# edogariu/artist-style-transfer

Measured on NVIDIA B200. Metric: train_images_per_sec_256, higher is better.
Workload: dtype bf16

## Files before the change

### artist_style_transfer_b200/csrc/common.cuh

```cuda
#pragma once
#include <cstring>
#include <cstdlib>
#include <cuda_runtime.h>
#include <cuda_bf16.h>
#include <cuda_fp16.h>
#include <stdint.h>
#include <stdio.h>
#include <atomic>

#include "../../include/ast.h"

namespace ast {

void set_error(const char* fmt, ...);
extern std::atomic<long long> g_launches;
inline void count_launch(int n = 1) { g_launches.fetch_add(n, std::memory_order_relaxed); }

enum Family {
  FAM_CONV_TC = 0, FAM_CONV_PX, FAM_CONV_WS, FAM_CONV_HX, FAM_CONV_SIMT, FAM_WGRAD_TC, FAM_WGRAD_THIN, FAM_WGRAD_SIMT, FAM_GRAM_TC,
  FAM_GRAM_SIMT, FAM_IN_APPLY, FAM_IN_BWD, FAM_IN_STATS, FAM_POOL, FAM_MSE, FAM_POINTWISE, FAM_OPTIM, FAM_CONV_ST, FAM_COUNT
};
void count_work(int family, double flops, double bytes);
inline double esize(const ast_image* im) { return im->dtype == AST_F32 ? 4.0 : (im->dtype == AST_U8 ? 1.0 : 2.0); }
inline double img_bytes(const ast_image* im) { return im ? (double)im->n * im->h * im->w * im->c * esize(im) : 0.0; }
// ... 62 lines not shown
  static constexpr int id = AST_BF16;
  __device__ static __forceinline__ float ld(const __nv_bfloat16* p) { return __bfloat162float(*p); }
  __device__ static __forceinline__ void st(__nv_bfloat16* p, float v) { *p = __float2bfloat16_rn(v); }
};

__device__ __forceinline__ __half f2h_sat(float v) { return __float2half_rn(fminf(fmaxf(v, -65504.f), 65504.f)); }
template <bool F16>
__device__ __forceinline__ unsigned pack2(float a, float b) {
  if (F16) { const __half2 h = __halves2half2(f2h_sat(a), f2h_sat(b)); return *reinterpret_cast<const unsigned*>(&h); }
  const __nv_bfloat162 h = __floats2bfloat162_rn(a, b);
  return *reinterpret_cast<const unsigned*>(&h);
}
__device__ __forceinline__ unsigned pack2_16(int dtype, float a, float b) { return dtype == AST_F16 ? pack2<true>(a, b) : pack2<false>(a, b); }
__device__ __forceinline__ float ld_elem(const Img& im, long long off) {
  if (im.dtype == AST_F32) return ((const float*)im.ptr)[off];
  if (im.dtype == AST_U8) return (float)((const unsigned char*)im.ptr)[off];
  if (im.dtype == AST_BF16) return __bfloat162float(((const __nv_bfloat16*)im.ptr)[off]);
  return __half2float(((const __half*)im.ptr)[off]);
}
__device__ __forceinline__ void st_elem(const Img& im, long long off, float v) {
  if (im.dtype == AST_F32) ((float*)im.ptr)[off] = v;
  else if (im.dtype == AST_BF16) ((__nv_bfloat16*)im.ptr)[off] = __float2bfloat16_rn(v);
  else if (im.dtype == AST_F16) ((__half*)im.ptr)[off] = f2h_sat(v);
  else ((unsigned char*)im.ptr)[off] = (unsigned char)__float2uint_rz(fminf(fmaxf(v, 0.f), 255.f));
}
__device__ __forceinline__ long long img_off(const Img& im, int n, int y, int x, int c) {
  return (long long)n * im.sn + (long long)y * im.sh + (long long)x * im.sw + (long long)c * im.sc;
}
__device__ __forceinline__ int reflect_idx(int i, int n) {
  if (i < 0) i = -i;
  if (i >= n) i = 2 * (n - 1) - i;
  return i;
}
template <typename F>
__device__ __forceinline__ void reflect_fold_border(int pad, int H, int W, int i, int j, F&& add) {
  const int r1 = (i >= 1 && i <= pad) ? pad - i : -1;
  const int r2 = (i <= H - 2 && i >= H - 1 - pad) ? pad + 2 * (H - 1) - i : -1;
  const int c1 = (j >= 1 && j <= pad) ? pad - j : -1;
  const int c2 = (j <= W - 2 && j >= W - 1 - pad) ? pad + 2 * (W - 1) - j : -1;
#pragma unroll
  for (int a_ = 0; a_ < 3; ++a_) {
    const int r = a_ == 0 ? i + pad : (a_ == 1 ? r1 : r2);
    if (r < 0) continue;
#pragma unroll
    for (int b_ = 0; b_ < 3; ++b_) {
      const int cc = b_ == 0 ? j + pad : (b_ == 1 ? c1 : c2);
      if (cc < 0 || (a_ == 0 && b_ == 0)) continue;
      add(r, cc);
    }
  }
}

__device__ __forceinline__ float warp_sum(float v) {
#pragma unroll
  for (int o = 16; o > 0; o >>= 1) v += __shfl_xor_sync(0xffffffffu, v, o);
  return v;
}

template <typename T> struct Vec16;
template <> struct Vec16<float> {
  static constexpr int N = 4;
  __device__ static __forceinline__ void load(const float* p, float* out) {
    float4 v = *reinterpret_cast<const float4*>(p);
    out[0] = v.x; out[1] = v.y; out[2] = v.z; out[3] = v.w;
  }
  __device__ static __forceinline__ void store(float* p, const float* in) {
    *reinterpret_cast<float4*>(p) = make_float4(in[0], in[1], in[2], in[3]);
  }
};
template <> struct Vec16<__nv_bfloat16> {
  static constexpr int N = 8;
  __device__ static __forceinline__ void load(const __nv_bfloat16* p, float* out) {
// ... 64 lines not shown
```

### artist_style_transfer_b200/csrc/norm.cu

```cuda
#include "tc_common.cuh"

namespace ast {

constexpr int NT = 256;

template <typename T>
__global__ void __launch_bounds__(NT)
in_stats_partial_kernel(Img x, float* __restrict__ ws, int nblk, int chunk) {
  constexpr int VEC = Vec16<T>::N;
  extern __shared__ float sm[];
  const int C = x.c, lanes = C / VEC, slots = NT / lanes;
  const int tid = threadIdx.x, lane = tid % lanes, slot = tid / lanes;
  const int n = blockIdx.y, blk = blockIdx.x;
  const int hw = x.h * x.w;
  const int pbeg = blk * chunk, pend = min(hw, pbeg + chunk);
  const T* base = (const T*)x.ptr + (long long)n * x.sn + lane * VEC;

  float k[VEC], s1[VEC], s2[VEC];
#pragma unroll
  for (int e = 0; e < VEC; ++e) { k[e] = 0.f; s1[e] = 0.f; s2[e] = 0.f; }
  int cnt = 0;
  if (slot < slots) {
    for (int p = pbeg + slot; p < pend; p += slots) {
      const int y = p / x.w, xx = p - y * x.w;
// ... 55 lines not shown
    rstd[n * C + c] = rsqrtf(qa / (float)hw + eps);
  }
}

__global__ void in_finalize_kernel(const double* __restrict__ sums, int total, double inv_hw, float eps,
                                   float* __restrict__ mean, float* __restrict__ rstd) {
  const int i = blockIdx.x * blockDim.x + threadIdx.x;
  if (i >= total) return;
  const double m = sums[2 * i] * inv_hw;
  const double var = fmax(sums[2 * i + 1] * inv_hw - m * m, 0.0);
  mean[i] = (float)m;
  rstd[i] = (float)(1.0 / sqrt(var + (double)eps));
}


constexpr int NS_CONSUMER_WARPS = 8;
constexpr int NS_CONSUMERS = NS_CONSUMER_WARPS * 32;
constexpr int NS_THREADS = NS_CONSUMERS + 32;
constexpr int NS_SLAB_MAX = 16384;
constexpr int NS_MAX_STAGES = 8;
constexpr int NS_SMEM_BUDGET = 100 * 1024;

struct Rows {
  char* ptr;
  long long sn;
  int sh;
};

struct NsShape {
  int C, H, W, pad;
  int nblk;
  int seg, nseg;
  int stages, slab_bytes;
};

template <typename T> struct NsVec;
template <> struct NsVec<float> {
  static constexpr int N = 4;
  __device__ static __forceinline__ void unpack(const uint4& r, float* v) {
    v[0] = __uint_as_float(r.x); v[1] = __uint_as_float(r.y); v[2] = __uint_as_float(r.z); v[3] = __uint_as_float(r.w);
  }
  __device__ static __forceinline__ uint4 pack(const float* v) {
    return make_uint4(__float_as_uint(v[0]), __float_as_uint(v[1]), __float_as_uint(v[2]), __float_as_uint(v[3]));
  }
};
template <> struct NsVec<__nv_bfloat16> {
  static constexpr int N = 8;
  __device__ static __forceinline__ void unpack(const uint4& r, float* v) {
    const unsigned w[4] = {r.x, r.y, r.z, r.w};
#pragma unroll
    for (int i = 0; i < 4; ++i) { v[2 * i] = __uint_as_float(w[i] << 16); v[2 * i + 1] = __uint_as_float(w[i] & 0xffff0000u); }
  }
  __device__ static __forceinline__ uint4 pack(const float* v) {
    uint4 r;
    __nv_bfloat162* h = reinterpret_cast<__nv_bfloat162*>(&r);
#pragma unroll
    for (int i = 0; i < 4; ++i) h[i] = __floats2bfloat162_rn(v[2 * i], v[2 * i + 1]);
    return r;
  }
};

template <int VEC>
__device__ __forceinline__ void ns_ldc(const float* __restrict__ p, float* v) {
#pragma unroll
  for (int e = 0; e < VEC; e += 4) {
    const float4 t = __ldg(reinterpret_cast<const float4*>(p + e));
// ... 86 lines not shown
  for (int k = 0; k < nunits; ++k) {
    const int s = k % sh.stages;
    const unsigned ph = (unsigned)(k / sh.stages) & 1u;
    const int oy = rbeg + k / sh.nseg, sg = k % sh.nseg;
    const int oa = sg * sh.seg, ob = min(OW, oa + sh.seg);
    int xa, xb;
    apply_span(oa, ob, sh.pad, sh.W, xa, xb);
    const unsigned xs = buf + s * stage_bytes + (unsigned)(c * (int)sizeof(T));
    const int orow = oy * (out.sh / VEC);
    mbar_wait(&full[s], ph);
    for (int ox = oa + slot; ox < ob; ox += slots) {
      const int j = reflect_idx(ox - sh.pad, sh.W) - xa;
      float v[VEC];
      NsVec<T>::unpack(lds128(xs + (unsigned)(j * C * (int)sizeof(T))), v);
#pragma unroll
      for (int e = 0; e < VEC; ++e) v[e] = fmaf(A[e], v[e], D[e]);
      if (res.ptr) {
        float r[VEC];
        NsVec<T>::unpack(lds128(xs + sh.slab_bytes + (unsigned)(j * C * (int)sizeof(T))), r);
#pragma unroll
        for (int e = 0; e < VEC; ++e) v[e] += r[e];
      }
      if (relu) {
#pragma unroll
        for (int e = 0; e < VEC; ++e) v[e] = fmaxf(v[e], 0.f);
      }
      oimg[orow + ox * lanes] = NsVec<T>::pack(v);
    }
    __syncwarp();
    if ((threadIdx.x & 31) == 0) mbar_arrive(&empty[s]);
  }
}

template <typename T, int VEC>
__device__ __forceinline__ void ns_fold_border(const T* gimg, int gsh, int C, int pad, int H, int W, int i, int j, float* g) {
  reflect_fold_border(pad, H, W, i, j, [&](int r, int cc) {
    float t[VEC];
    NsVec<T>::unpack(__ldg(reinterpret_cast<const uint4*>(gimg + (r * gsh + cc * C))), t);
#pragma unroll
    for (int e = 0; e < VEC; ++e) g[e] += t[e];
  });
}

template <typename T>
__device__ __forceinline__ void ns_bwd_produce(const Rows& x, const Rows& gpad, const Rows& gextra, const NsShape& sh, int n,
                                               int rbeg, int nunits, int k0, unsigned buf, int stage_bytes,
                                               unsigned long long* full, unsigned long long* empty) {
  const int C = sh.C;
  const int nslabs = 1 + (gpad.ptr ? 1 : 0) + (gextra.ptr ? 1 : 0);
  for (int k = 0; k < nunits; ++k) {
    const int s = (k0 + k) % sh.stages;
    const unsigned ph = (unsigned)((k0 + k) / sh.stages) & 1u;
    const int i = rbeg + k / sh.nseg, sg = k % sh.nseg;
    const int ja = sg * sh.seg, jb = min(sh.W, ja + sh.seg);
    const unsigned bytes = (unsigned)((jb - ja) * C * (int)sizeof(T));
    mbar_wait(&empty[s], ph ^ 1u);
    mbar_expect_tx(&full[s], bytes * nslabs);
    unsigned dst = buf + s * stage_bytes;
    bulk_load(dst, img_at<T>(x, n) + (i * x.sh + ja * C), bytes, &full[s]);
    dst += sh.slab_bytes;
    if (gpad.ptr) {
      bulk_load(dst, img_at<T>(gpad, n) + ((i + sh.pad) * gpad.sh + (ja + sh.pad) * C), bytes, &full[s]);
      dst += sh.slab_bytes;
    }
    if (gextra.ptr) bulk_load(dst, img_at<T>(gextra, n) + (i * gextra.sh + ja * C), bytes, &full[s]);
  }
}

template <typename T, int VEC>
__device__ __forceinline__ void ns_gprime(unsigned xs, unsigned gs, unsigned es, const T* gimg, int gsh, bool has_gextra,
                                          const NsShape& sh, bool brow, int i, int j, const float* A, const float* D,
                                          int relu, float* xv, float* g) {
  NsVec<T>::unpack(lds128(xs), xv);
  if (gimg) {
    NsVec<T>::unpack(lds128(gs), g);
    if (sh.pad > 0 && (brow || j <= sh.pad || j >= sh.W - 1 - sh.pad))
      ns_fold_border<T, VEC>(gimg, gsh, sh.C, sh.pad, sh.H, sh.W, i, j, g);
  } else {
#pragma unroll
    for (int e = 0; e < VEC; ++e) g[e] = 0.f;
  }
  if (has_gextra) {
    float t[VEC];
    NsVec<T>::unpack(lds128(es), t);
#pragma unroll
    for (int e = 0; e < VEC; ++e) g[e] += t[e];
  }
#pragma unroll
  for (int e = 0; e < VEC; ++e)
    if (relu && !(fmaf(A[e], xv[e], D[e]) > 0.f)) g[e] = 0.f;
}

enum NsMode { NS_STATS = 1, NS_APPLY = 2, NS_BOTH = 3 };

template <typename T, int MODE>
__global__ void __launch_bounds__(NS_THREADS, 2)
in_bwd_staged_kernel(Rows x, const float* __restrict__ mean, const float* __restrict__ rstd,
                     const float* __restrict__ gamma, const float* __restrict__ beta, Rows gpad, Rows gextra,
                     NsShape sh, int relu, float* __restrict__ s1, float* __restrict__ s2, int* __restrict__ arrive,
                     Rows dx, Rows gtotal) {
  constexpr int VEC = NsVec<T>::N;
  extern __shared__ unsigned char smem_raw[];
  __shared__ __align__(8) unsigned long long full[NS_MAX_STAGES], empty[NS_MAX_STAGES];
  const unsigned buf = (smem_u32(smem_raw) + 127u) & ~127u;
  ns_init(full, empty, sh.stages);
  const int n = blockIdx.y, C = sh.C;
  const int rbeg = (int)((long long)blockIdx.x * sh.H / sh.nblk), rend = (int)((long long)(blockIdx.x + 1) * sh.H / sh.nblk);
  const int nunits = (rend - rbeg) * sh.nseg;
  const int nslabs = 1 + (gpad.ptr ? 1 : 0) + (gextra.ptr ? 1 : 0);
  const int stage_bytes = nslabs * sh.slab_bytes;

  if (threadIdx.x >= NS_CONSUMERS) {
    if (threadIdx.x == NS_CONSUMERS) {
      ns_bwd_produce<T>(x, gpad, gextra, sh, n, rbeg, nunits, 0, buf, stage_bytes, full, empty);
      if (MODE == NS_BOTH) ns_bwd_produce<T>(x, gpad, gextra, sh, n, rbeg, nunits, nunits, buf, stage_bytes, full, empty);
    }
    return;
  }
  const int lanes = C / VEC, slots = NS_CONSUMERS / lanes;
  const int lane = threadIdx.x % lanes, slot = threadIdx.x / lanes;
  const int c = lane * VEC;
  float A[VEC], D[VEC];
  ns_fold_ad<VEC>(gamma, beta, mean, rstd, n, C, c, A, D);
  const T* const gimg = gpad.ptr ? img_at<T>(gpad, n) + c : nullptr;

  auto consume = [&](int k, int pos, auto&& f) {
    const int s = pos % sh.stages;
    const unsigned ph = (unsigned)(pos / sh.stages) & 1u;
    const int i = rbeg + k / sh.nseg, sg = k % sh.nseg;
    const int ja = sg * sh.seg, jb = min(sh.W, ja + sh.seg);
    const bool brow = sh.pad > 0 && (i <= sh.pad || i >= sh.H - 1 - sh.pad);
    const unsigned xs = buf + s * stage_bytes + (unsigned)(c * (int)sizeof(T));
    const unsigned gs = xs + sh.slab_bytes;
    const unsigned es = xs + (gpad.ptr ? 2 : 1) * sh.slab_bytes;
    mbar_wait(&full[s], ph);
    for (int j = ja + slot; j < jb; j += slots) {
      const unsigned poff = (unsigned)((j - ja) * C * (int)sizeof(T));
      float xv[VEC], g[VEC];
      ns_gprime<T, VEC>(xs + poff, gs + poff, es + poff, gimg, gpad.sh, gextra.ptr != nullptr, sh, brow, i, j, A, D, relu,
                        xv, g);
      f(j, xv, g);
    }
    __syncwarp();
    if ((threadIdx.x & 31) == 0) mbar_arrive(&empty[s]);
  };

  if (MODE & NS_STATS) {
    float t1[VEC], t2[VEC];
#pragma unroll
    for (int e = 0; e < VEC; ++e) { t1[e] = 0.f; t2[e] = 0.f; }
    for (int k = 0; k < nunits; ++k)
      consume(k, k, [&](int, const float* xv, const float* g) {
#pragma unroll
        for (int e = 0; e < VEC; ++e) { t1[e] += g[e]; t2[e] = fmaf(g[e], xv[e], t2[e]); }
      });
    float* r1 = reinterpret_cast<float*>(smem_raw + (buf - smem_u32(smem_raw)) +
                                         (MODE == NS_BOTH ? (size_t)sh.stages * stage_bytes : 0));
    float* r2 = r1 + slots * C;
    if (MODE == NS_STATS) {
      __syncwarp();
      asm volatile("bar.sync 1, %0;" ::"n"(NS_CONSUMERS) : "memory");
    }
#pragma unroll
    for (int e = 0; e < VEC; ++e) { r1[slot * C + c + e] = t1[e]; r2[slot * C + c + e] = t2[e]; }
    asm volatile("bar.sync 1, %0;" ::"n"(NS_CONSUMERS) : "memory");
    for (int cc = threadIdx.x; cc < C; cc += NS_CONSUMERS) {
      float u1 = 0.f, u2 = 0.f;
      for (int q = 0; q < slots; ++q) { u1 += r1[q * C + cc]; u2 += r2[q * C + cc]; }
      atomicAdd(s1 + n * C + cc, u1);
      atomicAdd(s2 + n * C + cc, rstd[n * C + cc] * (u2 - mean[n * C + cc] * u1));
    }
    if (MODE == NS_BOTH) {
      __threadfence();
      asm volatile("bar.sync 1, %0;" ::"n"(NS_CONSUMERS) : "memory");
      if (threadIdx.x == 0) {
        atomicAdd(arrive + n, 1);
        const volatile int* cnt = arrive + n;
        for (unsigned spin = 0; *cnt < sh.nblk; ++spin)
          if (spin > (1u << 28)) __trap();
        __threadfence();
      }
      asm volatile("bar.sync 1, %0;" ::"n"(NS_CONSUMERS) : "memory");
    }
  }

  if (MODE & NS_APPLY) {
    const float inv_hw = 1.f / (float)(sh.H * sh.W);
    float B[VEC], Cc[VEC];
    {
      float mu[VEC], rs[VEC];
      ns_ldc<VEC>(rstd + n * C + c, rs); ns_ldc<VEC>(mean + n * C + c, mu);
#pragma unroll
      for (int e = 0; e < VEC; ++e) {
        const float S1 = __ldcg(s1 + n * C + c + e), S2 = __ldcg(s2 + n * C + c + e);
        B[e] = -A[e] * rs[e] * S2 * inv_hw;
        Cc[e] = -A[e] * S1 * inv_hw - B[e] * mu[e];
      }
    }
    const int k0 = MODE == NS_BOTH ? nunits : 0;
    T* const dimg = img_at<T>(dx, n) + c;
    T* const timg = gtotal.ptr ? img_at<T>(gtotal, n) + c : nullptr;
    for (int k = 0; k < nunits; ++k) {
      const int i = rbeg + k / sh.nseg;
      const int drow = i * dx.sh, trow = i * gtotal.sh;
      consume(k, k0 + k, [&](int j, float* xv, const float* g) {
        if (timg) *reinterpret_cast<uint4*>(timg + (trow + j * C)) = NsVec<T>::pack(g);
#pragma unroll
        for (int e = 0; e < VEC; ++e) xv[e] = fmaf(A[e], g[e], fmaf(B[e], xv[e], Cc[e]));
        *reinterpret_cast<uint4*>(dimg + (drow + j * C)) = NsVec<T>::pack(xv);
      });
    }
  }
}

static int stats_blocks(int n, int hw, int slots) {
  int nblk = (4 * num_sms() + n - 1) / n;
  const int maxb = (hw + slots * 4 - 1) / (slots * 4);
  if (nblk > maxb) nblk = maxb;
  if (nblk < 1) nblk = 1;
  return nblk;
}

static bool nhwc_ok(const ast_image* x, int vec) {
  return x->sc == 1 && x->c % vec == 0 && x->sw % vec == 0 && x->sh % vec == 0 && x->sn % vec == 0;
}

static bool rows_ok(const ast_image* im, int vec) {
  return im->sc == 1 && im->sw == im->c && im->c % vec == 0 && im->sh % vec == 0 && im->sn % vec == 0 && im->sh >= 0 &&
         im->sn >= 0 && ((uintptr_t)im->ptr & 15) == 0 && (long long)im->h * im->sh < (1ll << 31);
}
static int staged_layout_check(const char* who, const ast_image* x, std::initializer_list<const ast_image*> tensors) {
  AST_CHECK_ARG(x->dtype == AST_F32 || x->dtype == AST_BF16, "%s: x must be fp32 or bf16 (dtype %d)", who, x->dtype);
  const int esz = x->dtype == AST_F32 ? 4 : 2, vec = 16 / esz;
  for (const ast_image* t : tensors) {
    if (!t) continue;
    AST_CHECK_ARG(t->dtype == x->dtype, "%s: every tensor must have the dtype of x (%d vs %d)", who, t->dtype, x->dtype);
    AST_CHECK_ARG(rows_ok(t, vec), "%s: needs NHWC with dense 16-byte aligned rows, < 2^31 elements per image (sc == 1, sw == c, C %% %d == 0; got "
                  "c=%d sw=%lld sc=%lld)", who, vec, t->c, (long long)t->sw, (long long)t->sc);
  }
  AST_CHECK_ARG(x->c > 0 && x->c * esz <= NS_SLAB_MAX / 8 && NS_CONSUMERS % (x->c / vec) == 0,
                "%s: C=%d is not supported", who, x->c);
  return 0;
}

static Rows to_rows(const ast_image* im) {
  Rows r;
  if (!im) { r.ptr = nullptr; r.sn = r.sh = 0; return r; }
  r.ptr = (char*)im->ptr; r.sn = im->sn; r.sh = (int)im->sh;
  return r;
}
static bool ns_plan(NsShape* sh, int n, int C, int H, int W, int pad, int rows_total, int width, int esz, int nslabs,
                    int slab_max = NS_SLAB_MAX, int budget = NS_SMEM_BUDGET) {
  sh->C = C; sh->H = H; sh->W = W; sh->pad = pad;
  const int seg_max = slab_max / (C * esz) - (width != W ? 2 * pad : 0);
  if (seg_max < 4 * pad + 1) return false;
  sh->nseg = (width + seg_max - 1) / seg_max;
  sh->seg = (width + sh->nseg - 1) / sh->nseg;
  sh->nseg = (width + sh->seg - 1) / sh->seg;
  const int slab_px = sh->seg + (width != W ? 2 * pad : 0);
  sh->slab_bytes = (slab_px * C * esz + 127) / 128 * 128;
  sh->stages = budget / (nslabs * sh->slab_bytes);
  if (sh->stages > NS_MAX_STAGES) sh->stages = NS_MAX_STAGES;
  if (sh->stages < 2) return false;
  int nb = (2 * num_sms()) / n;
  if (nb > rows_total) nb = rows_total;
  if (nb < 1) nb = 1;
  sh->nblk = nb;
  return true;
}

template <typename... KP, typename... A>
static int ns_launch(const char* who, int family, double bytes, void (*kernel)(KP...), dim3 grid, size_t smem,
                     bool cooperative, cudaStream_t s, A... args) {
  cudaError_t e = set_max_smem(kernel, smem);
  if (e == cudaSuccess && !cooperative) {
    e = launch_k(kernel, grid, NS_THREADS, smem, s, args...);
  } else if (e == cudaSuccess) {
    cudaLaunchConfig_t cfg;
    memset(&cfg, 0, sizeof(cfg));
    cfg.gridDim = grid; cfg.blockDim = dim3(NS_THREADS); cfg.dynamicSmemBytes = smem; cfg.stream = s;
    cudaLaunchAttribute attr;
    attr.id = cudaLaunchAttributeCooperative;
    attr.val.cooperative = 1;
    cfg.attrs = &attr; cfg.numAttrs = 1;
    e = cudaLaunchKernelEx(&cfg, kernel, static_cast<KP>(args)...);
  }
  if (e != cudaSuccess) { set_error("%s: launch failed: %s", who, cudaGetErrorString(e)); return (int)e; }
  count_launch();
  count_work(family, 0.0, bytes);
  AST_CUDA_LAUNCH_CHECK();
  return 0;
}

}

using namespace ast;
// ... 40 lines not shown
                                  const float* beta, const ast_image* residual, const ast_image* out, int32_t pad,
                                  int32_t relu, void* stream) {
  AST_CHECK_ARG(x && mean && rstd && gamma && beta && out, "ast_instnorm_apply: null argument");
  if (int e = staged_layout_check("ast_instnorm_apply", x, {x, out, residual})) return e;
  AST_CHECK_ARG(out->n == x->n && out->c == x->c && out->h == x->h + 2 * pad && out->w == x->w + 2 * pad,
                "ast_instnorm_apply: out must be (h+2p, w+2p)");
  AST_CHECK_ARG(pad < x->h && pad < x->w, "ast_instnorm_apply: pad too large for reflection");
  AST_CHECK_ARG(!residual || same_shape(residual, x), "ast_instnorm_apply: residual shape");
  if (x->n == 0) return 0;
  const int esz = x->dtype == AST_F32 ? 4 : 2, nslabs = residual ? 2 : 1;
  NsShape sh;
  AST_CHECK_ARG(ns_plan(&sh, x->n, x->c, x->h, x->w, pad, out->h, out->w, esz, nslabs),
                "ast_instnorm_apply: C=%d, pad=%d cannot be staged", x->c, pad);
  return ns_launch("ast_instnorm_apply", FAM_IN_APPLY, img_bytes(x) + img_bytes(out) + img_bytes(residual),
                   x->dtype == AST_F32 ? in_apply_staged_kernel<float> : in_apply_staged_kernel<__nv_bfloat16>,
                   dim3(sh.nblk, x->n), (size_t)sh.stages * nslabs * sh.slab_bytes + 128, false, (cudaStream_t)stream,
                   to_rows(x), mean, rstd, gamma, beta, to_rows(residual), to_rows(out), sh, relu);
}

extern "C" int ast_instnorm_bwd(const ast_image* x, const float* mean, const float* rstd, const float* gamma,
                                const float* beta, const ast_image* gpad, int32_t pad, const ast_image* gextra,
                                int32_t relu, float* s1, float* s2, int32_t* arrive, const ast_image* dx,
                                const ast_image* gtotal, void* stream) {
  AST_CHECK_ARG(x && mean && rstd && gamma && beta && s1 && s2 && arrive && dx, "ast_instnorm_bwd: null argument");
  AST_CHECK_ARG(relu == 0 || relu == 1, "ast_instnorm_bwd: relu must be 0 or 1 (got %d)", relu);
  if (int e = staged_layout_check("ast_instnorm_bwd", x, {x, gpad, gextra, dx, gtotal})) return e;
  AST_CHECK_ARG(!gpad || (gpad->n == x->n && gpad->c == x->c && gpad->h == x->h + 2 * pad && gpad->w == x->w + 2 * pad),
                "ast_instnorm_bwd: gpad must be (h+2p, w+2p)");
  AST_CHECK_ARG(!gextra || same_shape(gextra, x), "ast_instnorm_bwd: gextra shape");
  AST_CHECK_ARG(pad < x->h && pad < x->w, "ast_instnorm_bwd: pad too large");
  AST_CHECK_ARG(same_shape(dx, x), "ast_instnorm_bwd: dx shape");
  AST_CHECK_ARG(!gtotal || same_shape(gtotal, x), "ast_instnorm_bwd: gtotal shape");
  if (x->n == 0) return 0;
  const bool f32 = x->dtype == AST_F32;
  const int esz = f32 ? 4 : 2, vec = 16 / esz, nslabs = 1 + (gpad ? 1 : 0) + (gextra ? 1 : 0);
  const size_t scratch = 2 * (size_t)(NS_CONSUMERS / (x->c / vec)) * x->c * sizeof(float);
  const double bytes = 2.0 * img_bytes(x) + img_bytes(dx) + img_bytes(gtotal);
  cudaStream_t s = (cudaStream_t)stream;
  const Rows xr = to_rows(x), gp = to_rows(gpad), ge = to_rows(gextra), dxr = to_rows(dx), gt = to_rows(gtotal);
  NsShape sh;

  const double resident = (double)nslabs * x->n * x->h * x->w * x->c * esz;
  if (resident <= 104e6 &&
      ns_plan(&sh, x->n, x->c, x->h, x->w, pad, x->h, x->w, esz, nslabs, nslabs == 3 ? 8192 : NS_SLAB_MAX,
              NS_SMEM_BUDGET + 8192 - (int)scratch) &&
      (long long)sh.nblk * x->n <= 2ll * num_sms()) {
    const size_t smem = (size_t)sh.stages * nslabs * sh.slab_bytes + scratch + 128;
    if (smem <= 110 * 1024)
      return ns_launch("ast_instnorm_bwd", FAM_IN_BWD, bytes,
                       f32 ? in_bwd_staged_kernel<float, NS_BOTH> : in_bwd_staged_kernel<__nv_bfloat16, NS_BOTH>,
                       dim3(sh.nblk, x->n), smem, true, s, xr, mean, rstd, gamma, beta, gp, ge, sh, relu, s1, s2, arrive,
                       dxr, gt);
  }

  AST_CHECK_ARG(ns_plan(&sh, x->n, x->c, x->h, x->w, pad, x->h, x->w, esz, nslabs),
                "ast_instnorm_bwd: C=%d, pad=%d cannot be staged", x->c, pad);
  const size_t ring = (size_t)sh.stages * nslabs * sh.slab_bytes;
  if (int e = ns_launch("ast_instnorm_bwd", FAM_IN_BWD, 0.0,
                        f32 ? in_bwd_staged_kernel<float, NS_STATS> : in_bwd_staged_kernel<__nv_bfloat16, NS_STATS>,
                        dim3(sh.nblk, x->n), (ring > scratch ? ring : scratch) + 128, false, s, xr, mean, rstd, gamma,
                        beta, gp, ge, sh, relu, s1, s2, arrive, dxr, gt))
    return e;
  return ns_launch("ast_instnorm_bwd", FAM_IN_BWD, bytes,
                   f32 ? in_bwd_staged_kernel<float, NS_APPLY> : in_bwd_staged_kernel<__nv_bfloat16, NS_APPLY>,
                   dim3(sh.nblk, x->n), ring + 128, false, s, xr, mean, rstd, gamma, beta, gp, ge, sh, relu, s1, s2,
                   arrive, dxr, gt);
}
```

Baseline: 3455.

## Stage reflect-pad mirror rows in smem ring for instnorm backward

The instance-norm backward kernel used to fold reflect-padded gradient borders with scattered global __ldg loads. It now bulk-loads the padded gradient segment, including halo columns, plus the mirror rows into the TMA ring as extra stages, so the border fold reads shared memory. Rows are split across blocks by a weighted prefix that counts the extra mirror-row loads. The cross-lane stats reduction now uses warp shuffles to shrink the scratch area. The cost is more smem per stage, more ring stages consumed at border rows, and extra template variants.

```diff
diff --git a/artist_style_transfer_b200/csrc/common.cuh b/artist_style_transfer_b200/csrc/common.cuh
--- a/artist_style_transfer_b200/csrc/common.cuh
+++ b/artist_style_transfer_b200/csrc/common.cuh
@@ -118,12 +118,14 @@
   if (i >= n) i = 2 * (n - 1) - i;
   return i;
 }
+__device__ __forceinline__ int reflect_mirror_lo(int pad, int i) { return (i >= 1 && i <= pad) ? pad - i : -1; }
+__device__ __forceinline__ int reflect_mirror_hi(int pad, int n, int i) {
+  return (i <= n - 2 && i >= n - 1 - pad) ? pad + 2 * (n - 1) - i : -1;
+}
 template <typename F>
 __device__ __forceinline__ void reflect_fold_border(int pad, int H, int W, int i, int j, F&& add) {
-  const int r1 = (i >= 1 && i <= pad) ? pad - i : -1;
-  const int r2 = (i <= H - 2 && i >= H - 1 - pad) ? pad + 2 * (H - 1) - i : -1;
-  const int c1 = (j >= 1 && j <= pad) ? pad - j : -1;
-  const int c2 = (j <= W - 2 && j >= W - 1 - pad) ? pad + 2 * (W - 1) - j : -1;
+  const int r1 = reflect_mirror_lo(pad, i), r2 = reflect_mirror_hi(pad, H, i);
+  const int c1 = reflect_mirror_lo(pad, j), c2 = reflect_mirror_hi(pad, W, j);
 #pragma unroll
   for (int a_ = 0; a_ < 3; ++a_) {
     const int r = a_ == 0 ? i + pad : (a_ == 1 ? r1 : r2);
diff --git a/artist_style_transfer_b200/csrc/norm.cu b/artist_style_transfer_b200/csrc/norm.cu
--- a/artist_style_transfer_b200/csrc/norm.cu
+++ b/artist_style_transfer_b200/csrc/norm.cu
@@ -111,6 +111,7 @@
   int nblk;
   int seg, nseg;
   int stages, slab_bytes;
+  int gslab_bytes;
 };
 
 template <typename T> struct NsVec;
@@ -263,57 +264,95 @@
   }
 }
 
-template <typename T, int VEC>
-__device__ __forceinline__ void ns_fold_border(const T* gimg, int gsh, int C, int pad, int H, int W, int i, int j, float* g) {
-  reflect_fold_border(pad, H, W, i, j, [&](int r, int cc) {
-    float t[VEC];
-    NsVec<T>::unpack(__ldg(reinterpret_cast<const uint4*>(gimg + (r * gsh + cc * C))), t);
-#pragma unroll
-    for (int e = 0; e < VEC; ++e) g[e] += t[e];
-  });
+
+struct NsRing {
+  int s = 0;
+  unsigned ph = 0;
+  __device__ __forceinline__ NsRing take(int stages) {
+    const NsRing cur = *this;
+    if (++s == stages) { s = 0; ph ^= 1u; }
+    return cur;
+  }
+};
+
+template <typename F>
+__device__ __forceinline__ void ns_bwd_units(const NsShape& sh, bool has_g, int rbeg, int rend, F&& f) {
+  for (int i = rbeg; i < rend; ++i) {
+    const int r1 = has_g ? reflect_mirror_lo(sh.pad, i) : -1;
+    const int r2 = has_g ? reflect_mirror_hi(sh.pad, sh.H, i) : -1;
+    for (int sg = 0, ja = 0; sg < sh.nseg; ++sg) {
+      const int jb = sg + 1 == sh.nseg ? sh.W : (sg + 1) * sh.W / sh.nseg;
+      f(i, ja, jb, r1, r2);
+      ja = jb;
+    }
+  }
+}
+
+__device__ __forceinline__ int ns_bwd_row_split(const NsShape& sh, bool has_g, int b) {
+  if (!has_g || sh.pad == 0) return (int)((long long)b * sh.H / sh.nblk);
+  const int H = sh.H, pad = sh.pad;
+  auto prefix = [&](int i) {
+    return i + min(max(i - 1, 0), pad) + max(0, min(i, H - 1) - max(H - 1 - pad, 0));
+  };
+  const int target = (int)((long long)b * prefix(H) / sh.nblk);
+  int i = max(0, target - 2 * pad);
+  while (prefix(i) < target) ++i;
+  return i;
 }
 
 template <typename T>
 __device__ __forceinline__ void ns_bwd_produce(const Rows& x, const Rows& gpad, const Rows& gextra, const NsShape& sh, int n,
-                                               int rbeg, int nunits, int k0, unsigned buf, int stage_bytes,
+                                               int rbeg, int rend, NsRing& ring, unsigned buf, int stage_bytes,
                                                unsigned long long* full, unsigned long long* empty) {
   const int C = sh.C;
-  const int nslabs = 1 + (gpad.ptr ? 1 : 0) + (gextra.ptr ? 1 : 0);
-  for (int k = 0; k < nunits; ++k) {
-    const int s = (k0 + k) % sh.stages;
-    const unsigned ph = (unsigned)((k0 + k) / sh.stages) & 1u;
-    const int i = rbeg + k / sh.nseg, sg = k % sh.nseg;
-    const int ja = sg * sh.seg, jb = min(sh.W, ja + sh.seg);
+  const int nplain = 1 + (gextra.ptr ? 1 : 0);
+  ns_bwd_units(sh, gpad.ptr != nullptr, rbeg, rend, [&](int i, int ja, int jb, int r1, int r2) {
     const unsigned bytes = (unsigned)((jb - ja) * C * (int)sizeof(T));
-    mbar_wait(&empty[s], ph ^ 1u);
-    mbar_expect_tx(&full[s], bytes * nslabs);
-    unsigned dst = buf + s * stage_bytes;
-    bulk_load(dst, img_at<T>(x, n) + (i * x.sh + ja * C), bytes, &full[s]);
-    dst += sh.slab_bytes;
-    if (gpad.ptr) {
-      bulk_load(dst, img_at<T>(gpad, n) + ((i + sh.pad) * gpad.sh + (ja + sh.pad) * C), bytes, &full[s]);
-      dst += sh.slab_bytes;
-    }
-    if (gextra.ptr) bulk_load(dst, img_at<T>(gextra, n) + (i * gextra.sh + ja * C), bytes, &full[s]);
-  }
-}
-
-template <typename T, int VEC>
-__device__ __forceinline__ void ns_gprime(unsigned xs, unsigned gs, unsigned es, const T* gimg, int gsh, bool has_gextra,
-                                          const NsShape& sh, bool brow, int i, int j, const float* A, const float* D,
-                                          int relu, float* xv, float* g) {
-  NsVec<T>::unpack(lds128(xs), xv);
-  if (gimg) {
-    NsVec<T>::unpack(lds128(gs), g);
-    if (sh.pad > 0 && (brow || j <= sh.pad || j >= sh.W - 1 - sh.pad))
-      ns_fold_border<T, VEC>(gimg, gsh, sh.C, sh.pad, sh.H, sh.W, i, j, g);
+    const unsigned gbytes = (unsigned)((jb - ja + 2 * sh.pad) * C * (int)sizeof(T));
+    const T* const gseg = gpad.ptr ? img_at<T>(gpad, n) + ja * C : nullptr;
+#pragma unroll 1
+    for (int m = 0; m < 3; ++m) {
+      const int r = m == 0 ? r1 : m == 1 ? r2 : i + sh.pad;
+      if (r < 0) continue;
+      const NsRing q = ring.take(sh.stages);
+      mbar_wait(&empty[q.s], q.ph ^ 1u);
+      const unsigned dst = buf + q.s * stage_bytes;
+      if (m < 2) {
+        mbar_expect_tx(&full[q.s], gbytes);
+        bulk_load(dst + sh.slab_bytes, gseg + r * gpad.sh, gbytes, &full[q.s]);
+        continue;
+      }
+      mbar_expect_tx(&full[q.s], bytes * nplain + (gpad.ptr ? gbytes : 0u));
+      bulk_load(dst, img_at<T>(x, n) + (i * x.sh + ja * C), bytes, &full[q.s]);
+      if (gpad.ptr) bulk_load(dst + sh.slab_bytes, gseg + r * gpad.sh, gbytes, &full[q.s]);
+      if (gextra.ptr)
+        bulk_load(dst + sh.slab_bytes + sh.gslab_bytes, img_at<T>(gextra, n) + (i * gextra.sh + ja * C), bytes, &full[q.s]);
+    }
+  });
+}
+
+template <typename T, int VEC, bool FOLD>
+__device__ __forceinline__ void ns_gprime(unsigned xs, unsigned gs, unsigned m1, unsigned m2, unsigned es, bool has_g,
+                                          bool has_gextra, const NsShape& sh, bool brow, int i, int j, int ja,
+                                          const float* A, const float* D, int relu, float* xv, float* g) {
+  const unsigned pix = (unsigned)(sh.C * (int)sizeof(T));
+  NsVec<T>::unpack(lds128(xs + (unsigned)(j - ja) * pix), xv);
+  if (has_g) {
+    NsVec<T>::unpack(lds128(gs + (unsigned)(j + sh.pad - ja) * pix), g);
+    if (FOLD && (brow || j <= sh.pad || j >= sh.W - 1 - sh.pad))
+      reflect_fold_border(sh.pad, sh.H, sh.W, i, j, [&](int r, int cc) {
+        float t[VEC];
+        NsVec<T>::unpack(lds128((r == i + sh.pad ? gs : r < sh.pad ? m1 : m2) + (unsigned)(cc - ja) * pix), t);
+#pragma unroll
+        for (int e = 0; e < VEC; ++e) g[e] += t[e];
+      });
   } else {
 #pragma unroll
     for (int e = 0; e < VEC; ++e) g[e] = 0.f;
   }
   if (has_gextra) {
     float t[VEC];
-    NsVec<T>::unpack(lds128(es), t);
+    NsVec<T>::unpack(lds128(es + (unsigned)(j - ja) * pix), t);
 #pragma unroll
     for (int e = 0; e < VEC; ++e) g[e] += t[e];
   }
@@ -324,7 +363,11 @@
 
 enum NsMode { NS_STATS = 1, NS_APPLY = 2, NS_BOTH = 3 };
 
-template <typename T, int MODE>
+__host__ __device__ constexpr int ns_red_rows(int lanes) {
+  return lanes < 32 ? NS_CONSUMER_WARPS : NS_CONSUMERS / lanes;
+}
+
+template <typename T, int MODE, bool FOLD>
 __global__ void __launch_bounds__(NS_THREADS, 2)
 in_bwd_staged_kernel(Rows x, const float* __restrict__ mean, const float* __restrict__ rstd,
                      const float* __restrict__ gamma, const float* __restrict__ beta, Rows gpad, Rows gextra,
@@ -336,15 +379,15 @@
   const unsigned buf = (smem_u32(smem_raw) + 127u) & ~127u;
   ns_init(full, empty, sh.stages);
   const int n = blockIdx.y, C = sh.C;
-  const int rbeg = (int)((long long)blockIdx.x * sh.H / sh.nblk), rend = (int)((long long)(blockIdx.x + 1) * sh.H / sh.nblk);
-  const int nunits = (rend - rbeg) * sh.nseg;
-  const int nslabs = 1 + (gpad.ptr ? 1 : 0) + (gextra.ptr ? 1 : 0);
-  const int stage_bytes = nslabs * sh.slab_bytes;
+  const int rbeg = ns_bwd_row_split(sh, gpad.ptr != nullptr, blockIdx.x);
+  const int rend = ns_bwd_row_split(sh, gpad.ptr != nullptr, blockIdx.x + 1);
+  const int stage_bytes = sh.slab_bytes * (1 + (gextra.ptr ? 1 : 0)) + sh.gslab_bytes;
 
   if (threadIdx.x >= NS_CONSUMERS) {
     if (threadIdx.x == NS_CONSUMERS) {
-      ns_bwd_produce<T>(x, gpad, gextra, sh, n, rbeg, nunits, 0, buf, stage_bytes, full, empty);
-      if (MODE == NS_BOTH) ns_bwd_produce<T>(x, gpad, gextra, sh, n, rbeg, nunits, nunits, buf, stage_bytes, full, empty);
+      NsRing ring;
+      ns_bwd_produce<T>(x, gpad, gextra, sh, n, rbeg, rend, ring, buf, stage_bytes, full, empty);
+      if (MODE == NS_BOTH) ns_bwd_produce<T>(x, gpad, gextra, sh, n, rbeg, rend, ring, buf, stage_bytes, full, empty);
     }
     return;
   }
@@ -353,51 +396,65 @@
   const int c = lane * VEC;
   float A[VEC], D[VEC];
   ns_fold_ad<VEC>(gamma, beta, mean, rstd, n, C, c, A, D);
-  const T* const gimg = gpad.ptr ? img_at<T>(gpad, n) + c : nullptr;
-
-  auto consume = [&](int k, int pos, auto&& f) {
-    const int s = pos % sh.stages;
-    const unsigned ph = (unsigned)(pos / sh.stages) & 1u;
-    const int i = rbeg + k / sh.nseg, sg = k % sh.nseg;
-    const int ja = sg * sh.seg, jb = min(sh.W, ja + sh.seg);
-    const bool brow = sh.pad > 0 && (i <= sh.pad || i >= sh.H - 1 - sh.pad);
-    const unsigned xs = buf + s * stage_bytes + (unsigned)(c * (int)sizeof(T));
-    const unsigned gs = xs + sh.slab_bytes;
-    const unsigned es = xs + (gpad.ptr ? 2 : 1) * sh.slab_bytes;
-    mbar_wait(&full[s], ph);
+  const bool has_g = gpad.ptr != nullptr;
+
+  NsRing ring;
+  const unsigned coff = (unsigned)(c * (int)sizeof(T));
+  auto consume = [&](int i, int ja, int jb, int r1, int r2, auto&& f) {
+    NsRing q1, q2;
+    if (r1 >= 0) { q1 = ring.take(sh.stages); mbar_wait(&full[q1.s], q1.ph); }
+    if (r2 >= 0) { q2 = ring.take(sh.stages); mbar_wait(&full[q2.s], q2.ph); }
+    const NsRing q0 = ring.take(sh.stages);
+    const unsigned xs = buf + q0.s * stage_bytes + coff;
+    const unsigned gs = xs + sh.slab_bytes, es = gs + sh.gslab_bytes;
+    mbar_wait(&full[q0.s], q0.ph);
+    const bool brow = r1 >= 0 || r2 >= 0;
+    const unsigned m1 = buf + q1.s * stage_bytes + sh.slab_bytes + coff;
+    const unsigned m2 = buf + q2.s * stage_bytes + sh.slab_bytes + coff;
     for (int j = ja + slot; j < jb; j += slots) {
-      const unsigned poff = (unsigned)((j - ja) * C * (int)sizeof(T));
       float xv[VEC], g[VEC];
-      ns_gprime<T, VEC>(xs + poff, gs + poff, es + poff, gimg, gpad.sh, gextra.ptr != nullptr, sh, brow, i, j, A, D, relu,
-                        xv, g);
+      ns_gprime<T, VEC, FOLD>(xs, gs, m1, m2, es, has_g, gextra.ptr != nullptr, sh, brow, i, j, ja, A, D, relu, xv, g);
       f(j, xv, g);
     }
     __syncwarp();
-    if ((threadIdx.x & 31) == 0) mbar_arrive(&empty[s]);
+    if ((threadIdx.x & 31) == 0) {
+      if (r1 >= 0) mbar_arrive(&empty[q1.s]);
+      if (r2 >= 0) mbar_arrive(&empty[q2.s]);
+      mbar_arrive(&empty[q0.s]);
+    }
   };
 
   if (MODE & NS_STATS) {
     float t1[VEC], t2[VEC];
 #pragma unroll
     for (int e = 0; e < VEC; ++e) { t1[e] = 0.f; t2[e] = 0.f; }
-    for (int k = 0; k < nunits; ++k)
-      consume(k, k, [&](int, const float* xv, const float* g) {
+    ns_bwd_units(sh, has_g, rbeg, rend, [&](int i, int ja, int jb, int r1, int r2) {
+      consume(i, ja, jb, r1, r2, [&](int, const float* xv, const float* g) {
 #pragma unroll
         for (int e = 0; e < VEC; ++e) { t1[e] += g[e]; t2[e] = fmaf(g[e], xv[e], t2[e]); }
       });
+    });
+    for (int o = lanes; o < 32; o <<= 1)
+#pragma unroll
+      for (int e = 0; e < VEC; ++e) {
+        t1[e] += __shfl_xor_sync(0xffffffffu, t1[e], o);
+        t2[e] += __shfl_xor_sync(0xffffffffu, t2[e], o);
+      }
+    const int rows = ns_red_rows(lanes), row = lanes < 32 ? threadIdx.x / 32 : slot;
     float* r1 = reinterpret_cast<float*>(smem_raw + (buf - smem_u32(smem_raw)) +
                                          (MODE == NS_BOTH ? (size_t)sh.stages * stage_bytes : 0));
-    float* r2 = r1 + slots * C;
+    float* r2 = r1 + rows * C;
     if (MODE == NS_STATS) {
       __syncwarp();
       asm volatile("bar.sync 1, %0;" ::"n"(NS_CONSUMERS) : "memory");
     }
-#pragma unroll
-    for (int e = 0; e < VEC; ++e) { r1[slot * C + c + e] = t1[e]; r2[slot * C + c + e] = t2[e]; }
+    if (lanes >= 32 || (threadIdx.x & 31) < lanes)
+#pragma unroll
+      for (int e = 0; e < VEC; ++e) { r1[row * C + c + e] = t1[e]; r2[row * C + c + e] = t2[e]; }
     asm volatile("bar.sync 1, %0;" ::"n"(NS_CONSUMERS) : "memory");
     for (int cc = threadIdx.x; cc < C; cc += NS_CONSUMERS) {
       float u1 = 0.f, u2 = 0.f;
-      for (int q = 0; q < slots; ++q) { u1 += r1[q * C + cc]; u2 += r2[q * C + cc]; }
+      for (int q = 0; q < rows; ++q) { u1 += r1[q * C + cc]; u2 += r2[q * C + cc]; }
       atomicAdd(s1 + n * C + cc, u1);
       atomicAdd(s2 + n * C + cc, rstd[n * C + cc] * (u2 - mean[n * C + cc] * u1));
     }
@@ -428,20 +485,24 @@
         Cc[e] = -A[e] * S1 * inv_hw - B[e] * mu[e];
       }
     }
-    const int k0 = MODE == NS_BOTH ? nunits : 0;
     T* const dimg = img_at<T>(dx, n) + c;
     T* const timg = gtotal.ptr ? img_at<T>(gtotal, n) + c : nullptr;
-    for (int k = 0; k < nunits; ++k) {
-      const int i = rbeg + k / sh.nseg;
+    ns_bwd_units(sh, has_g, rbeg, rend, [&](int i, int ja, int jb, int r1, int r2) {
       const int drow = i * dx.sh, trow = i * gtotal.sh;
-      consume(k, k0 + k, [&](int j, float* xv, const float* g) {
+      consume(i, ja, jb, r1, r2, [&](int j, float* xv, const float* g) {
         if (timg) *reinterpret_cast<uint4*>(timg + (trow + j * C)) = NsVec<T>::pack(g);
 #pragma unroll
         for (int e = 0; e < VEC; ++e) xv[e] = fmaf(A[e], g[e], fmaf(B[e], xv[e], Cc[e]));
         *reinterpret_cast<uint4*>(dimg + (drow + j * C)) = NsVec<T>::pack(xv);
       });
-    }
-  }
+    });
+  }
+}
+
+template <int MODE>
+static auto ns_bwd_kernel(bool f32, bool fold) {
+  return f32 ? (fold ? in_bwd_staged_kernel<float, MODE, true> : in_bwd_staged_kernel<float, MODE, false>)
+             : (fold ? in_bwd_staged_kernel<__nv_bfloat16, MODE, true> : in_bwd_staged_kernel<__nv_bfloat16, MODE, false>);
 }
 
 static int stats_blocks(int n, int hw, int slots) {
@@ -481,18 +542,19 @@
   return r;
 }
 static bool ns_plan(NsShape* sh, int n, int C, int H, int W, int pad, int rows_total, int width, int esz, int nslabs,
-                    int slab_max = NS_SLAB_MAX, int budget = NS_SMEM_BUDGET) {
+                    int slab_max = NS_SLAB_MAX, int budget = NS_SMEM_BUDGET, int gslabs = 0, int min_stages = 2) {
   sh->C = C; sh->H = H; sh->W = W; sh->pad = pad;
   const int seg_max = slab_max / (C * esz) - (width != W ? 2 * pad : 0);
   if (seg_max < 4 * pad + 1) return false;
   sh->nseg = (width + seg_max - 1) / seg_max;
   sh->seg = (width + sh->nseg - 1) / sh->nseg;
-  sh->nseg = (width + sh->seg - 1) / sh->seg;
+  if (!gslabs) sh->nseg = (width + sh->seg - 1) / sh->seg;
   const int slab_px = sh->seg + (width != W ? 2 * pad : 0);
   sh->slab_bytes = (slab_px * C * esz + 127) / 128 * 128;
-  sh->stages = budget / (nslabs * sh->slab_bytes);
+  sh->gslab_bytes = gslabs ? ((sh->seg + 2 * pad) * C * esz + 127) / 128 * 128 : 0;
+  sh->stages = budget / ((nslabs - gslabs) * sh->slab_bytes + sh->gslab_bytes);
   if (sh->stages > NS_MAX_STAGES) sh->stages = NS_MAX_STAGES;
-  if (sh->stages < 2) return false;
+  if (sh->stages < min_stages) return false;
   int nb = (2 * num_sms()) / n;
   if (nb > rows_total) nb = rows_total;
   if (nb < 1) nb = 1;
@@ -599,37 +661,44 @@
   AST_CHECK_ARG(same_shape(dx, x), "ast_instnorm_bwd: dx shape");
   AST_CHECK_ARG(!gtotal || same_shape(gtotal, x), "ast_instnorm_bwd: gtotal shape");
   if (x->n == 0) return 0;
-  const bool f32 = x->dtype == AST_F32;
+  const bool f32 = x->dtype == AST_F32, fold = gpad && pad > 0;
   const int esz = f32 ? 4 : 2, vec = 16 / esz, nslabs = 1 + (gpad ? 1 : 0) + (gextra ? 1 : 0);
-  const size_t scratch = 2 * (size_t)(NS_CONSUMERS / (x->c / vec)) * x->c * sizeof(float);
+  const size_t scratch = 2 * (size_t)ns_red_rows(x->c / vec) * x->c * sizeof(float);
   const double bytes = 2.0 * img_bytes(x) + img_bytes(dx) + img_bytes(gtotal);
   cudaStream_t s = (cudaStream_t)stream;
   const Rows xr = to_rows(x), gp = to_rows(gpad), ge = to_rows(gextra), dxr = to_rows(dx), gt = to_rows(gtotal);
   NsShape sh;
+  const bool two_mirrors = gpad && pad > 0 && std::max(1, x->h - 1 - pad) <= std::min(pad, x->h - 2);
+  auto plan = [&](int slab_max, int budget) {
+    for (int cap = slab_max;; cap /= 2) {
+      if (ns_plan(&sh, x->n, x->c, x->h, x->w, pad, x->h, x->w, esz, nslabs, cap, budget, gpad ? 1 : 0,
+                  two_mirrors ? 3 : 2))
+        return true;
+      if (!two_mirrors || cap / 2 < 8 * x->c * esz) return false;
+    }
+  };
+  auto stage_bytes = [&] { return (size_t)sh.slab_bytes * (nslabs - (gpad ? 1 : 0)) + sh.gslab_bytes; };
 
   const double resident = (double)nslabs * x->n * x->h * x->w * x->c * esz;
-  if (resident <= 104e6 &&
-      ns_plan(&sh, x->n, x->c, x->h, x->w, pad, x->h, x->w, esz, nslabs, nslabs == 3 ? 8192 : NS_SLAB_MAX,
-              NS_SMEM_BUDGET + 8192 - (int)scratch) &&
+  if (resident <= 104e6 && plan(nslabs == 3 ? 8192 : NS_SLAB_MAX, NS_SMEM_BUDGET + 8192 - (int)scratch) &&
       (long long)sh.nblk * x->n <= 2ll * num_sms()) {
-    const size_t smem = (size_t)sh.stages * nslabs * sh.slab_bytes + scratch + 128;
+    const size_t smem = sh.stages * stage_bytes() + scratch + 128;
     if (smem <= 110 * 1024)
       return ns_launch("ast_instnorm_bwd", FAM_IN_BWD, bytes,
-                       f32 ? in_bwd_staged_kernel<float, NS_BOTH> : in_bwd_staged_kernel<__nv_bfloat16, NS_BOTH>,
+                       ns_bwd_kernel<NS_BOTH>(f32, fold),
                        dim3(sh.nblk, x->n), smem, true, s, xr, mean, rstd, gamma, beta, gp, ge, sh, relu, s1, s2, arrive,
                        dxr, gt);
   }
 
-  AST_CHECK_ARG(ns_plan(&sh, x->n, x->c, x->h, x->w, pad, x->h, x->w, esz, nslabs),
-                "ast_instnorm_bwd: C=%d, pad=%d cannot be staged", x->c, pad);
-  const size_t ring = (size_t)sh.stages * nslabs * sh.slab_bytes;
+  AST_CHECK_ARG(plan(NS_SLAB_MAX, NS_SMEM_BUDGET), "ast_instnorm_bwd: C=%d, pad=%d cannot be staged", x->c, pad);
+  const size_t ring = sh.stages * stage_bytes();
   if (int e = ns_launch("ast_instnorm_bwd", FAM_IN_BWD, 0.0,
-                        f32 ? in_bwd_staged_kernel<float, NS_STATS> : in_bwd_staged_kernel<__nv_bfloat16, NS_STATS>,
+                        ns_bwd_kernel<NS_STATS>(f32, fold),
                         dim3(sh.nblk, x->n), (ring > scratch ? ring : scratch) + 128, false, s, xr, mean, rstd, gamma,
                         beta, gp, ge, sh, relu, s1, s2, arrive, dxr, gt))
     return e;
   return ns_launch("ast_instnorm_bwd", FAM_IN_BWD, bytes,
-                   f32 ? in_bwd_staged_kernel<float, NS_APPLY> : in_bwd_staged_kernel<__nv_bfloat16, NS_APPLY>,
+                   ns_bwd_kernel<NS_APPLY>(f32, fold),
                    dim3(sh.nblk, x->n), ring + 128, false, s, xr, mean, rstd, gamma, beta, gp, ge, sh, relu, s1, s2,
                    arrive, dxr, gt);
 }
diff --git a/scratch/prof_in_bwd_step.py b/scratch/prof_in_bwd_step.py
--- /dev/null
+++ b/scratch/prof_in_bwd_step.py
@@ -0,0 +1,179 @@
+import argparse
+import os
+import subprocess
+import sys
+
+import torch
+
+sys.path.insert(0, os.path.dirname(os.path.dirname(os.path.abspath(__file__))))
+PEAK_GBS = 6464.9
+L2_BYTES = 126e6
+
+
+def card():
+    try:
+        q = subprocess.run(["nvidia-smi", "--query-gpu=name,power.limit,clocks.max.sm", "--format=csv,noheader"],
+                           capture_output=True, text=True, timeout=30).stdout.strip().splitlines()
+        return q[torch.cuda.current_device()] if q else "unknown"
+    except Exception as e:
+        return f"unknown ({e})"
+
+
+def record_step_calls(B=32, S=256):
+    import artist_style_transfer_b200 as ast
+    from artist_style_transfer_b200 import ops
+    dev = torch.device("cuda")
+    torch.manual_seed(2)
+    net = ast.StyleTransfer(device=dev, precision="fast")
+    vgg = ast.VGG16(vgg_path=None, precision="fast").to(dev)
+    style = ast.style_grams_single(vgg, torch.randint(0, 256, (3, S, S), device=dev).float(), B)
+    content = torch.randint(0, 256, (B, 3, S, S), device=dev).float()
+    calls, orig = [], ops.instnorm_bwd
+
+    def spy(x, mean, rstd, gamma, beta, gpad, pad, gextra, relu, dx, gtotal=None, s12=None, arrive=None):
+        cl = lambda t: None if t is None else t.detach().clone()
+        calls.append(dict(x=cl(x), mean=cl(mean), rstd=cl(rstd), gamma=cl(gamma), beta=cl(beta), gpad=cl(gpad),
+                          pad=int(pad), gextra=cl(gextra), relu=bool(relu), gtotal=gtotal is not None))
+        return orig(x, mean, rstd, gamma, beta, gpad, pad, gextra, relu, dx, gtotal, s12=s12, arrive=arrive)
+    ops.instnorm_bwd = spy
+    try:
+        ast.perceptual_step(net, vgg, content, style)
+        torch.cuda.synchronize()
+    finally:
+        ops.instnorm_bwd = orig
+    return calls
+
+
+def nbytes(t):
+    return 0 if t is None else t.numel() * t.element_size()
+
+
+def time_call(c, iters=20, reps=7):
+    from artist_style_transfer_b200 import ops, _lib
+    x, gpad, gextra = c["x"], c["gpad"], c["gextra"]
+    n, _, _, ch = x.shape
+    per_set = 2 * nbytes(x) + nbytes(gpad) + nbytes(gextra) + (nbytes(x) if c["gtotal"] else 0)
+    sets = max(2, int(3 * L2_BYTES / per_set) + 1)
+    bufs = []
+    for s in range(sets):
+        bufs.append(dict(x=x.clone(), gpad=None if gpad is None else gpad.clone(),
+                         gextra=None if gextra is None else gextra.clone(), dx=torch.empty_like(x),
+                         gt=torch.empty_like(x) if c["gtotal"] else None))
+    s12 = torch.zeros(iters, 2, n * ch, device="cuda")
+    arrive = torch.zeros(iters, n, dtype=torch.int32, device="cuda")
+
+    def run(i):
+        b = bufs[i % sets]
+        ops.instnorm_bwd(b["x"], c["mean"], c["rstd"], c["gamma"], c["beta"], b["gpad"], c["pad"], b["gextra"],
+                         c["relu"], b["dx"], b["gt"], s12=s12[i], arrive=arrive[i])
+    before = _lib.family_stats()
+    run(0)
+    launches = _lib.family_delta(before)["in_bwd"][0]
+    torch.cuda.synchronize()
+    graph, st = torch.cuda.CUDAGraph(), torch.cuda.Stream()
+    with torch.cuda.stream(st):
+        with torch.cuda.graph(graph, stream=st):
+            for i in range(iters):
+                run(i)
+    times = []
+    e0, e1 = torch.cuda.Event(enable_timing=True), torch.cuda.Event(enable_timing=True)
+    for r in range(reps + 1):
+        s12.zero_(); arrive.zero_()
+        torch.cuda.synchronize()
+        e0.record(); graph.replay(); e1.record()
+        torch.cuda.synchronize()
+        if r:
+            times.append(e0.elapsed_time(e1) * 1e3 / iters)
+    del graph
+    times.sort()
+    algo = nbytes(x) + nbytes(gpad) + nbytes(gextra) + nbytes(x) + (nbytes(x) if c["gtotal"] else 0)
+    return times[len(times) // 2], times[0], times[-1], launches, algo, sets
+
+
+def seeded_cases(calls):
+    out = []
+    step = [(*c["x"].shape, c["pad"], c["relu"], c["gextra"] is not None, c["x"].dtype) for c in calls]
+    for (n, h, w, ch, pad, relu, res, dt) in step + [(2, 64, 64, 128, 1, True, True, torch.bfloat16),
+                                             (1, 96, 80, 32, 4, True, False, torch.bfloat16),
+                                             (2, 3, 5, 32, 1, True, True, torch.bfloat16),
+                                             (1, 9, 12, 32, 4, False, True, torch.bfloat16),
+                                             (1, 40, 161, 128, 4, True, True, torch.bfloat16),
+                                             (2, 33, 263, 64, 4, True, False, torch.bfloat16),
+                                             (2, 64, 64, 128, 1, True, True, torch.float32),
+                                             (1, 7, 9, 64, 3, True, False, torch.float32),
+                                             (2, 20, 300, 32, 2, False, True, torch.float32)]:
+        g = torch.Generator(device="cuda").manual_seed(n * 1000 + h + w + ch + pad)
+        rn = lambda *s: torch.randn(*s, device="cuda", generator=g)
+        x = (rn(n, h, w, ch) * 2 + 0.5).to(dt)
+        xd = x.double()
+        mean = xd.mean(dim=(1, 2)).reshape(-1).float()
+        rstd = (xd.var(dim=(1, 2), unbiased=False) + 1e-5).rsqrt().reshape(-1).float()
+        out.append(dict(x=x, mean=mean, rstd=rstd, gamma=torch.rand(ch, device="cuda", generator=g) + 0.5,
+                        beta=rn(ch) * 0.3, gpad=rn(n, h + 2 * pad, w + 2 * pad, ch).to(dt), pad=pad,
+                        gextra=rn(n, h, w, ch).to(dt) if res else None, relu=relu, gtotal=True))
+    return out
+
+
+def dump(calls, d):
+    from artist_style_transfer_b200 import ops
+    os.makedirs(d, exist_ok=True)
+    for k, c in enumerate(seeded_cases(calls)):
+        x = c["x"]
+        n, _, _, ch = x.shape
+        dx, gt = torch.empty_like(x), torch.empty_like(x)
+        s12 = torch.zeros(2, n * ch, device="cuda")
+        arrive = torch.zeros(n, dtype=torch.int32, device="cuda")
+        ops.instnorm_bwd(x, c["mean"], c["rstd"], c["gamma"], c["beta"], c["gpad"], c["pad"], c["gextra"], c["relu"],
+                         dx, gt, s12=s12, arrive=arrive)
+        torch.save(dict(shape=tuple(x.shape), pad=c["pad"], gt=gt.cpu(), dx=dx.cpu(), s12=s12.cpu()),
+                   os.path.join(d, f"call{k:02d}.pt"))
+
+
+def compare(da, db):
+    ok = True
+    for f in sorted(os.listdir(da)):
+        a, b = torch.load(os.path.join(da, f)), torch.load(os.path.join(db, f))
+        same_g = torch.equal(a["gt"], b["gt"])
+        ad, bd = a["dx"].double(), b["dx"].double()
+        tol = ad.abs() * 2.0 ** -7 + 1e-5 * float(ad.abs().max())
+        dx_ok = not bool(((ad - bd).abs() > tol).any())
+        s_rel = float((a["s12"] - b["s12"]).norm() / (a["s12"].norm() + 1e-30))
+        good = same_g and dx_ok and s_rel < 1e-5
+        ok &= good
+        print(f"{f} {a['shape']} pad={a['pad']}: g' bit-identical {same_g}, dx within 2^-7 {dx_ok}, "
+              f"sums rel {s_rel:.1e} {'ok' if good else 'MISMATCH'}")
+    print("ALL OK" if ok else "MISMATCHES")
+    return ok
+
+
+def main():
+    ap = argparse.ArgumentParser()
+    ap.add_argument("--dump", metavar="DIR")
+    ap.add_argument("--compare", nargs=2, metavar="DIR")
+    ap.add_argument("--no-time", action="store_true")
+    args = ap.parse_args()
+    if args.compare:
+        sys.exit(0 if compare(*args.compare) else 1)
+    from artist_style_transfer_b200 import _lib
+    print(f"library {_lib.LIB_PATH}")
+    print(f"card: {card()}  (name, power.limit, clocks.max.sm)")
+    calls = record_step_calls()
+    print(f"{len(calls)} ops.instnorm_bwd calls in one B=32 256^2 fast step")
+    if not args.no_time:
+        print(f"{'#':>2} {'shape (N,H,W,C)':>20} {'pad':>3} {'relu':>4} {'gext':>4} {'gtot':>4} {'launch':>6} "
+              f"{'us':>7} {'min':>7} {'max':>7} {'MB':>7} {'GB/s':>6} {'frac':>5}")
+        tot_us, tot_launch = 0.0, 0
+        for k, c in enumerate(calls):
+            us, lo, hi, launches, algo, sets = time_call(c)
+            tot_us += us
+            tot_launch += launches
+            print(f"{k:2d} {str(tuple(c['x'].shape)):>20} {c['pad']:3d} {int(c['relu']):4d} {int(c['gextra'] is not None):4d} "
+                  f"{int(c['gtotal']):4d} {launches:6d} {us:7.1f} {lo:7.1f} {hi:7.1f} {algo / 1e6:7.1f} "
+                  f"{algo / us / 1e3:6.0f} {algo / us / 1e3 / PEAK_GBS:5.2f}", flush=True)
+        print(f"total {tot_us:.1f} us in {tot_launch} launches")
+    if args.dump:
+        dump(calls, args.dump)
+
+
+if __name__ == "__main__":
+    main()
```

Result: faster. 3515, median of 6 (+1.7%).
